# NVIDIA/makani

Hardware: AMD Instinct MI355X
Metric: SFNO train samples/sec at 721x1440x73ch (higher is better)
Workload: dtype bf16; 1 GPU; sfno_sc3_layers8_edim384; grid=721x1440, channels=73, global_batch=1, parallelism=dp1, spectral_arithmetic=x3, multistep_count=1, multistep_checkpoint=False, launch=hipGraph replay of the captured step, channel_gemm=hip (csrc/conv1x1.hip)

## Files before the change

### include/makani_amd.h

```cpp
#ifndef MAKANI_AMD_H
#define MAKANI_AMD_H

#ifdef __cplusplus
extern "C" {
#endif

#define MK_F32 0
#define MK_BF16 1

#define MK_EINVAL -1
#define MK_EUNSUP -2

#define MK_TRI_NONE 0
#define MK_TRI_ROW_GE 1
#define MK_TRI_K_GE 2
#define MK_TRI_ROW_LE 3
#define MK_TRI_K_LE 4

typedef struct MkGemm {
    const float* A;
    const float* B;
    float* C;
    long long a_batch, a_row, a_k;
    long long b_batch, b_col, b_k;
// ... 92 lines not shown

long long mk_spec_lp_blocks(int L, int M);
int mk_spec_lp_fwd(const float* S, const float* wgt, float* partial, int L, int M, long long R, int tri_off, int m_off,
                   float p, float w0, float w1, void* stream);
int mk_spec_lp_bwd(const float* S, const float* wgt, const float* g, float* dS, int L, int M, long long R, int tri_off,
                   int m_off, float p, float w0, float w1, void* stream);

int mk_spec_sep_mul(const float* x, const float* w, float* y, int L, int M, int Mw, int B, int Cp, int tri_off, int conj_w,
                    void* stream);
int mk_spec_sep_wgrad(const float* x, const float* gy, float* gw, int L, int M, int Mw, int B, int Cp, int tri_off, void* stream);
int mk_spec_diag_apply(const float* x, const float* w_c64, float* y, int L, int M, int B, int Cin, int Cout, int x_ld, int y_ld,
                       int y_pad, int tri_off, int dgrad, void* stream);
int mk_spec_diag_wgrad(const float* x, const float* gy, float* gw_c64, int L, int M, int B, int Cin, int Cout, int x_ld, int y_ld,
                       int tri_off, void* stream);

int mk_conv1x1_nn(const void* A, const void* X, void* Y, void* Ypre, const float* bias, const void* R, const void* G,
                  int M, int K, int lda, int B, long long N, int act, void* stream);
long long mk_conv1x1_wgrad_workspace(int M, int K, int B, long long N);
int mk_conv1x1_wgrad(const void* G, const void* X, float* dW, float* part, int M, int K, int B, long long N,
                     int accumulate, void* stream);
int mk_conv1x1_wgrad_fuses_bias(int M, int K, int B, long long N);
int mk_conv1x1_wgrad_bias(const void* G, const void* X, float* dW, float* dbias, float* part, int M, int K, int B, long long N,
                          int accumulate, void* stream);

int mk_adamw_step(float* p, const float* g, float* m, float* v, long long n, const float* grad_scale, float lr,
                  float beta1, float beta2, float eps, float weight_decay, int step, const float* step_state, void* stream);
int mk_adamw_advance(float* state, float beta1, float beta2, void* stream);
typedef struct MkAdamTensor {
    float* p;
    const float* g;
    float* m;
    float* v;
    long long n;
    void* p_bf16;
    void* p_bf16_t;
    int cols;
    int ld, ld_t;
} MkAdamTensor;
int mk_adamw_multi(const MkAdamTensor* tensors, int count, const float* grad_scale, float lr, float beta1, float beta2,
                   float eps, float weight_decay, int step, const float* step_state, void* stream);
long long mk_grad_norm_workspace(const MkAdamTensor* tensors, int count);
int mk_grad_clip_coef(const MkAdamTensor* tensors, int count, float max_norm, float* partial, float* out, void* stream);
long long mk_grad_norm_workspace_pre(const MkAdamTensor* tensors, int count, const MkAdamTensor* pre, int npre);
int mk_grad_clip_coef_pre(const MkAdamTensor* tensors, int count, const MkAdamTensor* pre, int npre, float max_norm, float* partial,
                          float* out, void* stream);

// ... 111 lines not shown
```

### makani_amd/_lib.py

```python
import ctypes as C
import os

import torch

_HERE = os.path.dirname(os.path.abspath(__file__))
LIB_PATH = os.environ.get("MAKANI_AMD_LIB") or os.path.join(_HERE, "libmakani_amd.so")

MK_F32, MK_BF16 = 0, 1
TRI_NONE, TRI_ROW_GE, TRI_K_GE, TRI_ROW_LE, TRI_K_LE = 0, 1, 2, 3, 4

c_ll, c_int, c_f, c_vp = C.c_longlong, C.c_int, C.c_float, C.c_void_p


class MkAdamTensor(C.Structure):
    _fields_ = [("p", C.c_void_p), ("g", C.c_void_p), ("m", C.c_void_p), ("v", C.c_void_p), ("n", C.c_longlong),
                ("p_bf16", C.c_void_p), ("p_bf16_t", C.c_void_p), ("cols", C.c_int), ("ld", C.c_int), ("ld_t", C.c_int)]


class MkGemm(C.Structure):
    _fields_ = [
        ("A", c_vp), ("B", c_vp), ("C", c_vp),
        ("a_batch", c_ll), ("a_row", c_ll), ("a_k", c_ll),
        ("b_batch", c_ll), ("b_col", c_ll), ("b_k", c_ll),
        ("c_batch", c_ll), ("c_row", c_ll), ("c_col", c_ll),
        ("a_inner", c_ll), ("b_inner", c_ll), ("c_inner", c_ll),
        ("a_im", c_ll), ("b_im", c_ll), ("c_im", c_ll),
        ("M", c_int), ("N", c_int), ("K", c_int), ("batch", c_int),
        ("inner", c_int), ("tri_mode", c_int), ("tri_off", c_int),
        ("conj_a", c_int), ("conj_b", c_int), ("beta", c_int),
    ]


MK_FFT_SEG_MAX = 8


class MkFftSeg(C.Structure):
    _fields_ = [("nw", c_int), ("nh", c_int), ("m_off", c_int * (MK_FFT_SEG_MAX + 1)), ("r_off", c_int * (MK_FFT_SEG_MAX + 1)),
                ("base", (c_ll * MK_FFT_SEG_MAX) * MK_FFT_SEG_MAX), ("xseg", c_int), ("x_stride", c_ll), ("x_nlat", c_int)]

# ... 24 lines not shown
    "mk_spec_sep_mul": ([c_vp, c_vp, c_vp, c_int, c_int, c_int, c_int, c_int, c_int, c_int, c_vp], c_int),
    "mk_spec_sep_wgrad": ([c_vp, c_vp, c_vp, c_int, c_int, c_int, c_int, c_int, c_int, c_vp], c_int),
    "mk_spec_diag_apply": ([c_vp, c_vp, c_vp, c_int, c_int, c_int, c_int, c_int, c_int, c_int, c_int, c_int, c_int, c_vp], c_int),
    "mk_spec_diag_wgrad": ([c_vp, c_vp, c_vp, c_int, c_int, c_int, c_int, c_int, c_int, c_int, c_int, c_vp], c_int),
    "mk_pointwise_chunks": ([c_ll, c_int, c_ll], c_int),
    "mk_plane_sums": ([c_vp, c_int, c_vp, c_vp, c_ll, c_ll, c_vp], c_int),
    "mk_instnorm_stats": ([c_vp, c_int, c_vp, c_vp, c_ll, c_ll, c_f, c_vp, c_f, c_vp], c_int),
    "mk_instnorm_merge": ([c_vp, c_vp, c_vp, c_ll, c_int, c_f, c_vp], c_int),
    "mk_instnorm_apply": ([c_vp, c_vp, c_int, c_vp, c_vp, c_vp, c_ll, c_int, c_ll, c_int, c_vp], c_int),
    "mk_instnorm_fused_chunks": ([c_ll, c_int, c_ll, c_int], c_int),
    "mk_instnorm_fwd_fused": ([c_vp, c_vp, c_int, c_vp, c_vp, c_vp, c_vp, c_vp, c_vp, c_ll, c_int, c_ll, c_f, c_int, c_vp], c_int),
    "mk_instnorm_bwd_fused": ([c_vp, c_vp, c_vp, c_int, c_vp, c_vp, c_vp, c_vp, c_vp, c_vp, c_vp, c_ll, c_int, c_ll, c_int, c_vp], c_int),
    "mk_instnorm_bwd": ([c_vp, c_vp, c_vp, c_int, c_vp, c_vp, c_vp, c_vp, c_vp, c_f, c_vp, c_vp, c_ll, c_int, c_ll, c_ll, c_int, c_int, c_vp], c_int),
    "mk_chan_layernorm_chunks": ([c_int, c_ll], c_int),
    "mk_chan_layernorm_fwd": ([c_vp, c_int, c_vp, c_int, c_vp, c_vp, c_vp, c_int, c_int, c_ll, c_f, c_vp], c_int),
    "mk_chan_layernorm_bwd": ([c_vp, c_int, c_vp, c_int, c_vp, c_vp, c_vp, c_int, c_int, c_ll, c_vp], c_int),
    "mk_chan_layernorm_wgrad": ([c_vp, c_int, c_vp, c_int, c_vp, c_vp, c_int, c_int, c_ll, c_vp], c_int),
    "mk_bias_gelu_fwd": ([c_vp, c_vp, c_vp, c_int, c_ll, c_int, c_ll, c_vp], c_int),
    "mk_conv1x1_nn": ([c_vp, c_vp, c_vp, c_vp, c_vp, c_vp, c_vp, c_int, c_int, c_int, c_int, c_ll, c_int, c_vp], c_int),
    "mk_conv1x1_wgrad_workspace": ([c_int, c_int, c_int, c_ll], c_ll),
    "mk_conv1x1_wgrad": ([c_vp, c_vp, c_vp, c_vp, c_int, c_int, c_int, c_ll, c_int, c_vp], c_int),
    "mk_conv1x1_wgrad_fuses_bias": ([c_int, c_int, c_int, c_ll], c_int),
    "mk_conv1x1_wgrad_bias": ([c_vp, c_vp, c_vp, c_vp, c_vp, c_int, c_int, c_int, c_ll, c_int, c_vp], c_int),
    "mk_adamw_step": ([c_vp, c_vp, c_vp, c_vp, c_ll, c_vp, c_f, c_f, c_f, c_f, c_f, c_int, c_vp, c_vp], c_int),
    "mk_adamw_advance": ([c_vp, c_f, c_f, c_vp], c_int),
    "mk_bias_gelu_bwd": ([c_vp, c_vp, c_vp, c_vp, c_vp, c_vp, c_int, c_ll, c_int, c_ll, c_vp], c_int),
    "mk_adamw_multi": ([c_vp, c_int, c_vp, c_f, c_f, c_f, c_f, c_f, c_int, c_vp, c_vp], c_int),
    "mk_instnorm_fwd": ([c_vp, c_vp, c_int, c_vp, c_vp, c_vp, c_vp, c_vp, c_vp, c_f, c_ll, c_int, c_ll, c_f, c_int, c_vp], c_int),
    "mk_grad_norm_workspace": ([c_vp, c_int], c_ll),
    "mk_grad_clip_coef": ([c_vp, c_int, c_f, c_vp, c_vp, c_vp], c_int),
    "mk_grad_norm_workspace_pre": ([c_vp, c_int, c_vp, c_int], c_ll),
    "mk_grad_clip_coef_pre": ([c_vp, c_int, c_vp, c_int, c_f, c_vp, c_vp, c_vp], c_int),
    "mk_spec_lp_blocks": ([c_int, c_int], c_ll),
    "mk_spec_lp_fwd": ([c_vp, c_vp, c_vp, c_int, c_int, c_ll, c_int, c_int, c_f, c_f, c_f, c_vp], c_int),
    "mk_spec_lp_bwd": ([c_vp, c_vp, c_vp, c_vp, c_int, c_int, c_ll, c_int, c_int, c_f, c_f, c_f, c_vp], c_int),
    "mk_crps_chunks": ([c_ll], c_int),
    "mk_crps": ([c_vp, c_int, c_vp, c_int, c_vp, c_vp, c_vp, c_vp, c_vp, c_int, c_int, c_int, c_ll, c_int, c_f, c_f, c_int, c_vp, c_vp], c_int),
    "mk_crps_complex": ([c_vp, c_vp, c_vp, c_vp, c_vp, c_vp, c_vp, c_int, c_int, c_int, c_ll, c_f, c_int, c_vp], c_int),
    "mk_escore_sums_workspace": ([c_int, c_int, c_int, c_ll, c_int, c_int], c_ll),
    "mk_escore_sums": ([c_vp, c_int, c_vp, c_vp, c_vp, c_vp, c_vp, c_int, c_int, c_int, c_ll, c_int, c_int, c_f, c_vp], c_int),
    "mk_escore_finish": ([c_vp, c_vp, c_int, c_vp, c_vp, c_int, c_int, c_int, c_int, c_int, c_f, c_f, c_f, c_f, c_vp], c_int),
    "mk_escore_grad": ([c_vp, c_int, c_vp, c_vp, c_vp, c_vp, c_vp, c_vp, c_int, c_int, c_int, c_int, c_ll, c_int, c_int, c_f, c_vp], c_int),
    "mk_mmd_finish": ([c_vp, c_vp, c_vp, c_int, c_int, c_int, c_int, c_f, c_f, c_vp], c_int),
    "mk_amse_sums": ([c_vp, c_vp, c_vp, c_vp, c_ll, c_int, c_int, c_int, c_int, c_vp], c_int),
    "mk_amse_grad": ([c_vp, c_vp, c_vp, c_vp, c_vp, c_vp, c_ll, c_int, c_int, c_int, c_int, c_vp], c_int),
    "mk_ens_nll_chunks": ([c_ll], c_int),
# ... 124 lines not shown
```

### makani_amd/csrc/conv1x1.hip

```cpp
#include <stdlib.h>
#include <type_traits>

#include "common.h"
#include "conv1x1_plan.h"

#ifndef MK_ASTAT_DIAG
#define MK_ASTAT_DIAG 0
#endif
#if MK_ASTAT_DIAG
__device__ unsigned long long g_astat_diag[16];
#define MK_AS_STAMP(k)                                              \
    do {                                                            \
        const unsigned long long t_ = __builtin_readcyclecounter(); \
        dg[k] += t_ - tprev;                                        \
        tprev = t_;                                                 \
    } while (0)
#else
#define MK_AS_STAMP(k)
#endif

namespace {

typedef __bf16 bf16x8 __attribute__((ext_vector_type(8)));
typedef __attribute__((address_space(3))) s16x4 lds_s16x4;
// ... 1364 lines not shown
    for (int i = 0; i < 2; ++i)
#pragma unroll
        for (int j = 0; j < 2; ++j) {
            const int c = c0 + wn * 64 + j * 32 + l31;
#pragma unroll
            for (int r = 0; r < 16; ++r) {
                const int m = m0 + wm * 64 + i * 32 + (r & 3) + 8 * (r >> 2) + 4 * lh;
                if (m < p.M && c < p.K) out[(long long)m * p.K + c] = acc[i][j][r];
            }
        }
}

struct ConvWgR {
    const u16* P;
    const u16* Q;
    float* part;
    int RP, RQ, B, S, slabs, qslabs;
    int ldo;
    long long N;
    long long chunk;
    float* bias_part;
};


template <int WP, int WQ, int WTP, int WTQ, bool SWAP>
__global__ __launch_bounds__(512, 2) void conv_wgrad_ring_kernel(const ConvWgR p) {
#if defined(__HIP_DEVICE_COMPILE__)
    static_assert(WP * WQ == 8, "8 waves");
    constexpr int TP = WP * WTP * 32, TQ = WQ * WTQ * 32;
    constexpr int BK = 64;
    constexpr int STAGE = (TP + TQ) * 128;
    constexpr int NI = (TP + TQ) / 64;
    constexpr int NIP = TP / 64;
    static_assert(TP % 64 == 0 && TQ == 384, "row groups; Q is fetched by 2 x 3 DMA pieces per wave");
    __shared__ __attribute__((aligned(1024))) unsigned char smem[2 * STAGE];

    const int bid = xcd_remap(blockIdx.x, gridDim.x);
    const int slab = bid % p.slabs;
    const int qs = (bid / p.slabs) % p.qslabs;
    const int q0 = qs * TQ;
    const int sp = bid / (p.slabs * p.qslabs);
    const int splits_per_b = p.S / p.B;
    const int b = sp / splits_per_b;
    const long long nbeg = (long long)(sp % splits_per_b) * p.chunk;
    const long long nend = min(p.N, nbeg + p.chunk);
    const int nk = nbeg < nend ? (int)((nend - nbeg + BK - 1) / BK) : 0;

    const int tid = threadIdx.x, lane = tid & 63, wave = tid >> 6;
    const int wp = wave / WQ, wq = wave % WQ;
    const int l31 = lane & 31, lh = lane >> 5;

    const int c_log = (lane & 7) ^ ((((wave & 1) << 2) + (lane >> 4)) & 7);
    const unsigned rowbytes = (unsigned)(p.N * 2);
    unsigned voff[NI];
#pragma unroll
    for (int i = 0; i < NI; ++i) {
        const int rg = wave + 8 * i;
        int row;
        if (i < NIP) row = min(rg * 8 + (lane >> 3), p.RP - 1 - slab * TP);
        else row = min((rg - TP / 8) * 8 + (lane >> 3), p.RQ - 1 - q0);
        voff[i] = (unsigned)row * rowbytes + (unsigned)c_log * 16u;
    }
    const v4i_t rsP = make_rsrc(p.P + ((long long)b * p.RP + slab * TP) * p.N);
    const v4i_t rsQ = make_rsrc(p.Q + ((long long)b * p.RQ + q0) * p.N);
// ... 87 lines not shown
            const int m = SWAP ? q0 + (wq * WTQ + i) * 32 + l31 : slab * TP + (wp * WTP + i) * 32 + l31;
            if (lh == 0 && m < RG) p.bias_part[((long long)sp * NSH + bshare) * RG + m] = tot;
        }
    }

    float* out = p.part + (long long)sp * ((long long)(SWAP ? p.RQ : p.RP) * p.ldo);
#pragma unroll
    for (int i = 0; i < WTP; ++i)
#pragma unroll
        for (int j = 0; j < WTQ; ++j) {
            const int prow0 = slab * TP + (wp * WTP + i) * 32, qrow0 = q0 + (wq * WTQ + j) * 32;
#pragma unroll
            for (int r = 0; r < 16; ++r) {
                const int rr = (r & 3) + 8 * (r >> 2) + 4 * lh;
                const int m = SWAP ? qrow0 + rr : prow0 + rr;
                const int k = SWAP ? prow0 + l31 : qrow0 + l31;
                const bool ok = SWAP ? (m < p.RQ && k < p.RP) : (m < p.RP && k < p.RQ);
                if (ok) out[(long long)m * p.ldo + k] = acc[i][j][r];
            }
        }
#endif
}

__global__ void reduce_splits(const float* __restrict__ part, float* __restrict__ out, long long n, int S, int accumulate) {
    const long long i = (long long)blockIdx.x * blockDim.x + threadIdx.x;
    if (i >= n) return;
    float s = accumulate ? out[i] : 0.f;
    int k = 0;
    for (; k + 8 <= S; k += 8) {
        float v[8];
#pragma unroll
        for (int u = 0; u < 8; ++u) v[u] = part[(long long)(k + u) * n + i];
#pragma unroll
        for (int u = 0; u < 8; ++u) s += v[u];
    }
    for (; k < S; ++k) s += part[(long long)k * n + i];
    out[i] = s;
}

__global__ void reduce_splits4(const float4* __restrict__ part, float4* __restrict__ out, long long n4, int S, int accumulate) {
    const long long i = (long long)blockIdx.x * blockDim.x + threadIdx.x;
    if (i >= n4) return;
    float4 s = accumulate ? out[i] : make_float4(0.f, 0.f, 0.f, 0.f);
    int k = 0;
    for (; k + 8 <= S; k += 8) {
        float4 v[8];
#pragma unroll
        for (int u = 0; u < 8; ++u) v[u] = part[(long long)(k + u) * n4 + i];
#pragma unroll
        for (int u = 0; u < 8; ++u) s.x += v[u].x, s.y += v[u].y, s.z += v[u].z, s.w += v[u].w;
    }
    for (; k < S; ++k) {
        const float4 v = part[(long long)k * n4 + i];
        s.x += v.x, s.y += v.y, s.z += v.z, s.w += v.w;
    }
    out[i] = s;
}

}

#if MK_ASTAT_DIAG
extern "C" int mk_astat_diag_read(unsigned long long* out, int reset) {
    if (hipMemcpyFromSymbol(out, HIP_SYMBOL(g_astat_diag), sizeof(unsigned long long) * 16) != hipSuccess) return 1;
    if (reset) {
        unsigned long long z[16] = {};
        if (hipMemcpyToSymbol(HIP_SYMBOL(g_astat_diag), z, sizeof(z)) != hipSuccess) return 1;
    }
    return 0;
}
#endif

static int env_int(const char* name) {
    const char* e = getenv(name);
    return e ? atoi(e) : -1;
}

extern "C" int mk_conv1x1_nn(const void* A, const void* X, void* Y, void* Ypre, const float* bias, const void* R,
                             const void* G, int M, int K, int lda, int B, long long N, int act, void* stream) {
    MK_REQUIRE(A && X && Y, "conv1x1_nn: null pointer");
// ... 50 lines not shown
        const long long tn = (N + 255) / 256;
        const long long nt = (long long)tm * tn * B;
        const unsigned grid = (unsigned)(nt < 256 ? nt : 256);
        if (bm == 384) hipLaunchKernelGGL((conv_nn_ring_kernel<6>), dim3(grid), dim3(512), 0, s, p, tm, tn, nt);
        else if (bm == 256) hipLaunchKernelGGL((conv_nn_ring_kernel<4>), dim3(grid), dim3(512), 0, s, p, tm, tn, nt);
        else hipLaunchKernelGGL((conv_nn_ring_kernel<3>), dim3(grid), dim3(512), 0, s, p, tm, tn, nt);
        break;
    }
    case ConvNnKernel::tile: {
        constexpr int BM = 128;
        const int tm = (M + BM - 1) / BM;
        const int BN = N >= (1ll << 19) ? 256 : 128;
        const long long tn = (N + BN - 1) / BN;
        const long long nb = (long long)tm * tn * B;
        MK_REQUIRE(nb < (1ll << 31), "conv1x1_nn: grid too large");
        if (BN == 256) hipLaunchKernelGGL((conv_nn_kernel<BM, 256, 1, 64, 2>), dim3((unsigned)nb), dim3(NT), 0, s, p, tm, tn);
        else hipLaunchKernelGGL((conv_nn_kernel<BM, 128, 1, 64, 3>), dim3((unsigned)nb), dim3(NT), 0, s, p, tm, tn);
        break;
    }
    }
    return mk_check_launch("mk_conv1x1_nn");
}

namespace {
struct WgPlan {
    bool ring;
    bool swap;
    int tp;
    int slabs;
    int qslabs;
    long long S;
    long long chunk;
};

WgPlan wgrad_plan(int M, int K, int B, long long N) {
    WgPlan pl{};
    const int big = M > K ? M : K, small = M > K ? K : M;
    if (big >= 96 && N * 2 * 384 < (1ll << 31) && N >= 2048) {
        pl.ring = true;
        int q, pr;
        if (big <= 384) { q = big; pr = small; }
        else if (small <= 384) { q = small; pr = big; }
        else { q = big; pr = small; }
        const bool q_is_x = (K == q) && !(M == q && M > K);
        pl.swap = !q_is_x;
        pl.tp = (pr > 192 && pr % 256 != 192 && (pr % 192 != 0 || pr % 256 == 0)) ? 256 : 192;
        if (pr <= 192) pl.tp = 192;
        pl.slabs = (pr + pl.tp - 1) / pl.tp;
        pl.qslabs = (q + 383) / 384;
        long long per_b = 256 / ((long long)pl.slabs * pl.qslabs * B);
        if (per_b < 1) per_b = 1;
        const long long maxs = (N + 511) / 512;
        if (per_b > maxs) per_b = maxs;
        long long chunk = ((N + per_b - 1) / per_b + 63) / 64 * 64;
        per_b = (N + chunk - 1) / chunk;
        pl.chunk = chunk;
        pl.S = per_b * B;
        return pl;
    }
    const int tiles = ((M + 127) / 128) * ((K + 127) / 128);
    long long per_b = 1024 / ((long long)tiles * B);
    if (per_b < 1) per_b = 1;
    const long long maxs = (N + 2047) / 2048;
    if (per_b > maxs) per_b = maxs;
    long long chunk = (N + per_b - 1) / per_b;
    chunk = (chunk + 127) / 128 * 128;
    pl.chunk = chunk;
    pl.S = per_b * B;
    return pl;
}
}

extern "C" long long mk_conv1x1_wgrad_workspace(int M, int K, int B, long long N) {
    const WgPlan pl = wgrad_plan(M, K, B, N);
    return pl.S * (long long)M * K + pl.S * (long long)M;
}

extern "C" int mk_conv1x1_wgrad_fuses_bias(int M, int K, int B, long long N) {
    return wgrad_plan(M, K, B, N).ring ? 1 : 0;
}

static int conv1x1_wgrad_impl(const void* G, const void* X, float* dW, float* dbias, float* part, int M, int K, int B, long long N,
                              int accumulate, void* stream);

extern "C" int mk_conv1x1_wgrad(const void* G, const void* X, float* dW, float* part, int M, int K, int B, long long N,
                                int accumulate, void* stream) {
    return conv1x1_wgrad_impl(G, X, dW, nullptr, part, M, K, B, N, accumulate, stream);
}

extern "C" int mk_conv1x1_wgrad_bias(const void* G, const void* X, float* dW, float* dbias, float* part, int M, int K, int B,
                                     long long N, int accumulate, void* stream) {
    MK_REQUIRE(dbias, "conv1x1_wgrad_bias: null pointer");
    MK_REQUIRE(wgrad_plan(M, K, B, N).ring, "conv1x1_wgrad_bias: this shape runs the tile kernel, which does not form the bias gradient");
    return conv1x1_wgrad_impl(G, X, dW, dbias, part, M, K, B, N, accumulate, stream);
}

static int conv1x1_wgrad_impl(const void* G, const void* X, float* dW, float* dbias, float* part, int M, int K, int B, long long N,
                              int accumulate, void* stream) {
    MK_REQUIRE(G && X && dW && part, "conv1x1_wgrad: null pointer");
    MK_REQUIRE(M > 0 && K > 0 && B > 0 && N > 0 && (N % 8) == 0, "conv1x1_wgrad: bad shape");
    const WgPlan pl = wgrad_plan(M, K, B, N);
    hipStream_t s = (hipStream_t)stream;
    if (pl.ring) {
        ConvWgR p{};
        p.P = (const u16*)(pl.swap ? X : G);
        p.Q = (const u16*)(pl.swap ? G : X);
        p.RP = pl.swap ? K : M;
        p.RQ = pl.swap ? M : K;
        p.part = part, p.B = B, p.S = (int)pl.S, p.slabs = pl.slabs, p.qslabs = pl.qslabs, p.ldo = K, p.N = N, p.chunk = pl.chunk;
        p.bias_part = dbias ? part + pl.S * (long long)M * K : nullptr;
        const dim3 grid((unsigned)(pl.slabs * pl.qslabs * pl.S)), blk(512);
        if (pl.tp == 256) {
            if (pl.swap) hipLaunchKernelGGL((conv_wgrad_ring_kernel<2, 4, 4, 3, true>), grid, blk, 0, s, p);
            else hipLaunchKernelGGL((conv_wgrad_ring_kernel<2, 4, 4, 3, false>), grid, blk, 0, s, p);
        } else {
            if (pl.swap) hipLaunchKernelGGL((conv_wgrad_ring_kernel<2, 4, 3, 3, true>), grid, blk, 0, s, p);
            else hipLaunchKernelGGL((conv_wgrad_ring_kernel<2, 4, 3, 3, false>), grid, blk, 0, s, p);
        }
    } else {
        const int tm = (M + 127) / 128, tk = (K + 127) / 128;
        ConvWg p{(const u16*)G, (const u16*)X, part, M, K, B, (int)pl.S, N, pl.chunk};
        hipLaunchKernelGGL(conv_wgrad_kernel<128>, dim3((unsigned)(tm * tk * pl.S)), dim3(NT), 0, s, p, tm, tk);
    }
    const long long n = (long long)M * K;
    if (n % 4 == 0 && (((uintptr_t)part | (uintptr_t)dW) & 15) == 0)
        hipLaunchKernelGGL(reduce_splits4, dim3((unsigned)((n / 4 + 255) / 256)), dim3(256), 0, s, (const float4*)part, (float4*)dW,
                           n / 4, (int)pl.S, accumulate);
    else
        hipLaunchKernelGGL(reduce_splits, dim3((unsigned)((n + 255) / 256)), dim3(256), 0, s, part, dW, n, (int)pl.S, accumulate);
    if (dbias)
        hipLaunchKernelGGL(reduce_splits, dim3((unsigned)((M + 255) / 256)), dim3(256), 0, s, part + pl.S * n, dbias, (long long)M,
                           (int)pl.S, 0);
    return mk_check_launch("mk_conv1x1_wgrad");
}
```

### makani_amd/csrc/conv1x1_plan.h

```cpp
#pragma once

enum class ConvNnKernel {
    astat73,
    astat2,
    astat1,
    ring,
    tile
};

inline ConvNnKernel conv_nn_plan(int M, int K, int lda, int B, long long N, bool pre, bool has_r, bool has_g, int astat2_env) {
    const bool stationary = M >= 256 && (long long)M * N * 2 < (1ll << 31) && N >= 64 && !(has_r && has_g);
    if (stationary && lda == 80 && K > 64 && K <= 80 && (long long)K * N * 2 < (1ll << 32) && !((has_r || has_g) && pre))
        return ConvNnKernel::astat73;
    const bool small_ring = M == 384 && (long long)B * N <= 32768 && !pre && astat2_env != 1;
    if (stationary && K == 384 && !small_ring) return astat2_env == 0 ? ConvNnKernel::astat1 : ConvNnKernel::astat2;
    if (K >= 64 && M >= 192 && N * 2 * 64 < (1ll << 31) && (long long)M * lda * 2 < (1ll << 31) && N >= 256) return ConvNnKernel::ring;
    return ConvNnKernel::tile;
}

inline int conv_nn_ring_rows(int M, int K, int B, long long N, bool has_epilogue, int ring384_env) {
    const int rows = ((M % 256 == 0) || M > 576) ? 256 : 192;
    const long long tiles384 = ((N + 255) / 256) * B;
    if (rows == 192 && M > 192 && M <= 384 && K >= 512 && !has_epilogue && tiles384 >= 256 && ring384_env != 0) return 384;
    return rows;
}
```

### makani_amd/ops.py

```python
import ctypes as C
import os
import weakref
from dataclasses import dataclass

import numpy as np
import torch

from . import _lib
from ._lib import MkGemm, check, dtype_code, lib, ptr, stream
from . import legendre as _leg


def round4(n: int) -> int:
    return (n + 3) // 4 * 4


GEMM_MODE = os.environ.get("MAKANI_AMD_GEMM", "auto")
if GEMM_MODE not in ("auto", "x6", "x3", "fp32"):
    raise ValueError(f"MAKANI_AMD_GEMM={GEMM_MODE!r}: expected auto, x6, x3 or fp32")


def gemm_mode() -> str:
    if GEMM_MODE != "auto":
        return GEMM_MODE
# ... 985 lines not shown
    return y, ypre


def conv1x1_wgrad(g: torch.Tensor, x: torch.Tensor, want_bias: bool = False):
    B, M, H, W = g.shape
    K = x.shape[1]
    N = H * W
    g, x = g.contiguous(), x.contiguous()
    nws = lib().mk_conv1x1_wgrad_workspace(M, K, B, N)
    part = torch.empty((nws,), dtype=torch.float32, device=g.device)
    dW = torch.empty((M, K), dtype=torch.float32, device=g.device)
    fused = want_bias and bool(lib().mk_conv1x1_wgrad_fuses_bias(M, K, B, N))
    with _timed(f"conv1x1_wgrad_m{M}_k{K}_n{N}", flops=2.0 * B * M * K * N, nbytes=2.0 * B * N * (M + K)):
        if fused:
            db = torch.empty((M,), dtype=torch.float32, device=g.device)
            check(lib().mk_conv1x1_wgrad_bias(ptr(g), ptr(x), ptr(dW), ptr(db), ptr(part), M, K, B, N, 0, stream()), "mk_conv1x1_wgrad_bias")
        else:
            check(lib().mk_conv1x1_wgrad(ptr(g), ptr(x), ptr(dW), ptr(part), M, K, B, N, 0, stream()), "mk_conv1x1_wgrad")
    if not want_bias:
        return dW
    return dW, (db if fused else _sum_planes(g))


def _sum_planes(t: torch.Tensor) -> torch.Tensor:
    if not (t.is_cuda and t.dim() == 4 and t.dtype in (torch.bfloat16, torch.float32)):
        raise RuntimeError("makani_amd ops need 4-d bf16 / fp32 GPU tensors (the HIP path has no CPU fallback)")
    t = t.contiguous()
    B, Cc, H, W = t.shape
    sums = torch.empty((2, B * Cc), dtype=torch.float32, device=t.device)
    check(lib().mk_plane_sums(ptr(t), dtype_code(t), ptr(sums), ptr(_ws(B * Cc, H * W, t.dtype, t.device)), B * Cc, H * W,
                              stream()), "mk_plane_sums")
    return _batch_sum(sums, B, Cc)[0]


class Conv1x1Fn(torch.autograd.Function):

    @staticmethod
    def forward(ctx, x, weight, bias, residual):
        M, K = weight.shape[0], weight.shape[1]
        A, At = weight_operands(weight, need_t=ctx.needs_input_grad[0])
        y, _ = conv1x1_nn(A, K, x, bias=bias, residual=residual)
        ctx.save_for_backward(x, weight, At)
        ctx.has_bias = bias is not None
        ctx.has_res = residual is not None
        return y

# ... 22 lines not shown
class ConvGeluConvFn(torch.autograd.Function):

    @staticmethod
    def forward(ctx, x, w1, b1, w2, b2):
        H1, K = w1.shape[0], w1.shape[1]
        M = w2.shape[0]
        A1, A1t = weight_operands(w1, need_t=ctx.needs_input_grad[0])
        A2, A2t = weight_operands(w2, need_t=True)
        h, a1 = conv1x1_nn(A1, K, x, bias=b1, act=True, want_pre=True)
        y, _ = conv1x1_nn(A2, H1, h, bias=b2)
        ctx.save_for_backward(x, w1, w2, a1, h, A1t, A2t)
        ctx.has_b = (b1 is not None, b2 is not None)
        return y

    @staticmethod
    def backward(ctx, gy):
        x, w1, w2, a1, h, A1t, A2t = ctx.saved_tensors
        H1, K = w1.shape[0], w1.shape[1]
        M = w2.shape[0]
        gy = gy.contiguous()
        ga1, _ = conv1x1_nn(A2t, M, gy, gelu_grad_of=a1)
        gw2 = gb2 = gw1 = gb1 = None
        want_b2, want_b1 = ctx.has_b[1] and ctx.needs_input_grad[4], ctx.has_b[0] and ctx.needs_input_grad[2]
        if ctx.needs_input_grad[3] and want_b2:
            gw2, gb2 = conv1x1_wgrad(gy, h, want_bias=True)
            gw2 = gw2.view_as(w2)
        else:
            gw2 = conv1x1_wgrad(gy, h).view_as(w2) if ctx.needs_input_grad[3] else None
            gb2 = _sum_planes(gy) if want_b2 else None
        if ctx.needs_input_grad[1] and want_b1:
            gw1, gb1 = conv1x1_wgrad(ga1, x, want_bias=True)
            gw1 = gw1.view_as(w1)
        else:
            gw1 = conv1x1_wgrad(ga1, x).view_as(w1) if ctx.needs_input_grad[1] else None
            gb1 = _sum_planes(ga1) if want_b1 else None
        gx = None
        if ctx.needs_input_grad[0]:
            gx, _ = conv1x1_nn(A1t, H1, ga1)
        return gx, gw1, gb1, gw2, gb2


def want_bf16_shadow(param):
    param._mk_want_bf16 = True


def _shadow_valid(weight):
    return (getattr(weight, "_mk_shadow", None) is not None and getattr(weight, "_mk_shadow_version", -1) == weight._version
            and getattr(weight, "_mk_shadow_ptr", 0) == weight.data_ptr() and weight._mk_shadow.device == weight.device)


def cast_weight(weight, dtype):
    if dtype == weight.dtype:
        return weight
    if dtype == torch.bfloat16 and _shadow_valid(weight):
        K = weight.numel() // weight.shape[0]
        sh = weight._mk_shadow
        return sh.view(weight.shape) if sh.shape[1] == K else sh[:, :K]
    return weight.to(dtype)
# ... 245 lines not shown
```

Before: 27.68 samples/s.

## Batch both MLP weight-gradient GEMMs into one grouped ring kernel launch

Adds a grouped weight-gradient entry point that puts the two conv1x1 wgrad problems of the MLP backward into a single ring-kernel grid. Each block finds its problem and tile from a flattened tile index, and the split count is planned over the combined tile total. The split reductions for weights and biases are merged into one multi-segment reduce kernel. The aim is fewer launches and better occupancy for small per-problem grids, at the cost of a shared split plan and a larger workspace.

```diff
diff --git a/include/makani_amd.h b/include/makani_amd.h
--- a/include/makani_amd.h
+++ b/include/makani_amd.h
@@ -138,6 +138,16 @@
 int mk_conv1x1_wgrad_fuses_bias(int M, int K, int B, long long N);
 int mk_conv1x1_wgrad_bias(const void* G, const void* X, float* dW, float* dbias, float* part, int M, int K, int B, long long N,
                           int accumulate, void* stream);
+typedef struct MkWgradProblem {
+    const void* G;
+    const void* X;
+    float* dW;
+    float* dbias;
+    int M, K;
+    int accumulate;
+} MkWgradProblem;
+long long mk_conv1x1_wgrad_multi_workspace(const MkWgradProblem* probs, int n, int B, long long N);
+int mk_conv1x1_wgrad_multi(const MkWgradProblem* probs, int n, float* part, int B, long long N, void* stream);
 
 int mk_adamw_step(float* p, const float* g, float* m, float* v, long long n, const float* grad_scale, float lr,
                   float beta1, float beta2, float eps, float weight_decay, int step, const float* step_state, void* stream);
diff --git a/makani_amd/_lib.py b/makani_amd/_lib.py
--- a/makani_amd/_lib.py
+++ b/makani_amd/_lib.py
@@ -15,6 +15,11 @@
 class MkAdamTensor(C.Structure):
     _fields_ = [("p", C.c_void_p), ("g", C.c_void_p), ("m", C.c_void_p), ("v", C.c_void_p), ("n", C.c_longlong),
                 ("p_bf16", C.c_void_p), ("p_bf16_t", C.c_void_p), ("cols", C.c_int), ("ld", C.c_int), ("ld_t", C.c_int)]
+
+
+class MkWgradProblem(C.Structure):
+    _fields_ = [("G", C.c_void_p), ("X", C.c_void_p), ("dW", C.c_void_p), ("dbias", C.c_void_p), ("M", C.c_int), ("K", C.c_int),
+                ("accumulate", C.c_int)]
 
 
 class MkGemm(C.Structure):
@@ -85,6 +90,8 @@
     "mk_conv1x1_wgrad": ([c_vp, c_vp, c_vp, c_vp, c_int, c_int, c_int, c_ll, c_int, c_vp], c_int),
     "mk_conv1x1_wgrad_fuses_bias": ([c_int, c_int, c_int, c_ll], c_int),
     "mk_conv1x1_wgrad_bias": ([c_vp, c_vp, c_vp, c_vp, c_vp, c_int, c_int, c_int, c_ll, c_int, c_vp], c_int),
+    "mk_conv1x1_wgrad_multi_workspace": ([C.POINTER(MkWgradProblem), c_int, c_int, c_ll], c_ll),
+    "mk_conv1x1_wgrad_multi": ([C.POINTER(MkWgradProblem), c_int, c_vp, c_int, c_ll, c_vp], c_int),
     "mk_adamw_step": ([c_vp, c_vp, c_vp, c_vp, c_ll, c_vp, c_f, c_f, c_f, c_f, c_f, c_int, c_vp, c_vp], c_int),
     "mk_adamw_advance": ([c_vp, c_f, c_f, c_vp], c_int),
     "mk_bias_gelu_bwd": ([c_vp, c_vp, c_vp, c_vp, c_vp, c_vp, c_int, c_ll, c_int, c_ll, c_vp], c_int),
diff --git a/makani_amd/csrc/conv1x1.hip b/makani_amd/csrc/conv1x1.hip
--- a/makani_amd/csrc/conv1x1.hip
+++ b/makani_amd/csrc/conv1x1.hip
@@ -1410,9 +1410,23 @@
     float* bias_part;
 };
 
+struct ConvWgProb {
+    const u16* P;
+    const u16* Q;
+    float* part;
+    float* bias_part;
+    int RP, RQ, slabs, qslabs, ldo, swap;
+};
+struct ConvWgM {
+    ConvWgProb pr[WG_MULTI_MAX];
+    int n, T, B, S;
+    long long N;
+    long long chunk;
+};
+
 
 template <int WP, int WQ, int WTP, int WTQ, bool SWAP>
-__global__ __launch_bounds__(512, 2) void conv_wgrad_ring_kernel(const ConvWgR p) {
+__device__ __forceinline__ void conv_wgrad_ring_tile(const ConvWgR& p, unsigned char* smem, const int slab, const int qs, const int sp) {
 #if defined(__HIP_DEVICE_COMPILE__)
     static_assert(WP * WQ == 8, "8 waves");
     constexpr int TP = WP * WTP * 32, TQ = WQ * WTQ * 32;
@@ -1421,13 +1435,8 @@
     constexpr int NI = (TP + TQ) / 64;
     constexpr int NIP = TP / 64;
     static_assert(TP % 64 == 0 && TQ == 384, "row groups; Q is fetched by 2 x 3 DMA pieces per wave");
-    __shared__ __attribute__((aligned(1024))) unsigned char smem[2 * STAGE];
-
-    const int bid = xcd_remap(blockIdx.x, gridDim.x);
-    const int slab = bid % p.slabs;
-    const int qs = (bid / p.slabs) % p.qslabs;
+
     const int q0 = qs * TQ;
-    const int sp = bid / (p.slabs * p.qslabs);
     const int splits_per_b = p.S / p.B;
     const int b = sp / splits_per_b;
     const long long nbeg = (long long)(sp % splits_per_b) * p.chunk;
@@ -1561,39 +1570,90 @@
 #endif
 }
 
-__global__ void reduce_splits(const float* __restrict__ part, float* __restrict__ out, long long n, int S, int accumulate) {
-    const long long i = (long long)blockIdx.x * blockDim.x + threadIdx.x;
-    if (i >= n) return;
-    float s = accumulate ? out[i] : 0.f;
-    int k = 0;
-    for (; k + 8 <= S; k += 8) {
-        float v[8];
-#pragma unroll
-        for (int u = 0; u < 8; ++u) v[u] = part[(long long)(k + u) * n + i];
-#pragma unroll
-        for (int u = 0; u < 8; ++u) s += v[u];
-    }
-    for (; k < S; ++k) s += part[(long long)k * n + i];
-    out[i] = s;
-}
-
-__global__ void reduce_splits4(const float4* __restrict__ part, float4* __restrict__ out, long long n4, int S, int accumulate) {
-    const long long i = (long long)blockIdx.x * blockDim.x + threadIdx.x;
-    if (i >= n4) return;
-    float4 s = accumulate ? out[i] : make_float4(0.f, 0.f, 0.f, 0.f);
-    int k = 0;
-    for (; k + 8 <= S; k += 8) {
-        float4 v[8];
-#pragma unroll
-        for (int u = 0; u < 8; ++u) v[u] = part[(long long)(k + u) * n4 + i];
-#pragma unroll
-        for (int u = 0; u < 8; ++u) s.x += v[u].x, s.y += v[u].y, s.z += v[u].z, s.w += v[u].w;
-    }
-    for (; k < S; ++k) {
-        const float4 v = part[(long long)k * n4 + i];
-        s.x += v.x, s.y += v.y, s.z += v.z, s.w += v.w;
-    }
-    out[i] = s;
+template <int WTP>
+__global__ __launch_bounds__(512, 2) void conv_wgrad_ring_kernel(const ConvWgM a) {
+#if defined(__HIP_DEVICE_COMPILE__)
+    constexpr int STAGE = (2 * WTP * 32 + 384) * 128;
+    __shared__ __attribute__((aligned(1024))) unsigned char smem[2 * STAGE];
+    const int bid = xcd_remap(blockIdx.x, gridDim.x);
+    int t = bid % a.T;
+    const int sp = bid / a.T;
+    int i = 0;
+    for (; i + 1 < a.n; ++i) {
+        const int nt = a.pr[i].slabs * a.pr[i].qslabs;
+        if (t < nt) break;
+        t -= nt;
+    }
+    const ConvWgProb& q = a.pr[i];
+    ConvWgR p;
+    p.P = q.P, p.Q = q.Q, p.part = q.part, p.bias_part = q.bias_part;
+    p.RP = q.RP, p.RQ = q.RQ, p.slabs = q.slabs, p.qslabs = q.qslabs, p.ldo = q.ldo;
+    p.B = a.B, p.S = a.S, p.N = a.N, p.chunk = a.chunk;
+    const int slab = __builtin_amdgcn_readfirstlane(t % q.slabs), qs = __builtin_amdgcn_readfirstlane(t / q.slabs);
+    if (q.swap) conv_wgrad_ring_tile<2, 4, WTP, 3, true>(p, smem, slab, qs, sp);
+    else conv_wgrad_ring_tile<2, 4, WTP, 3, false>(p, smem, slab, qs, sp);
+#endif
+}
+
+struct RedSeg {
+    const float* part;
+    float* out;
+    long long n;
+    int vec, accumulate;
+    unsigned blk0;
+};
+struct RedArgs {
+    RedSeg seg[2 * WG_MULTI_MAX];
+    int nseg, S;
+};
+
+__global__ __launch_bounds__(256) void reduce_splits_multi(const RedArgs a) {
+    int g = 0;
+    while (g + 1 < a.nseg && blockIdx.x >= a.seg[g + 1].blk0) ++g;
+    const RedSeg& sg = a.seg[g];
+    const long long i = (long long)(blockIdx.x - sg.blk0) * 256 + threadIdx.x;
+    if (i >= sg.n) return;
+    const int S = a.S;
+    if (sg.vec) {
+        const float4* part = (const float4*)sg.part;
+        float4* out = (float4*)sg.out;
+        const long long n4 = sg.n;
+        float4 s = sg.accumulate ? out[i] : make_float4(0.f, 0.f, 0.f, 0.f);
+        int k = 0;
+        for (; k + 8 <= S; k += 8) {
+            float4 v[8];
+#pragma unroll
+            for (int u = 0; u < 8; ++u) v[u] = part[(long long)(k + u) * n4 + i];
+#pragma unroll
+            for (int u = 0; u < 8; ++u) s.x += v[u].x, s.y += v[u].y, s.z += v[u].z, s.w += v[u].w;
+        }
+        for (; k < S; ++k) {
+            const float4 v = part[(long long)k * n4 + i];
+            s.x += v.x, s.y += v.y, s.z += v.z, s.w += v.w;
+        }
+        out[i] = s;
+    } else {
+        const float* part = sg.part;
+        const long long n = sg.n;
+        float s = sg.accumulate ? sg.out[i] : 0.f;
+        int k = 0;
+        for (; k + 8 <= S; k += 8) {
+            float v[8];
+#pragma unroll
+            for (int u = 0; u < 8; ++u) v[u] = part[(long long)(k + u) * n + i];
+#pragma unroll
+            for (int u = 0; u < 8; ++u) s += v[u];
+        }
+        for (; k < S; ++k) s += part[(long long)k * n + i];
+        sg.out[i] = s;
+    }
+}
+
+inline void red_add(RedArgs& a, unsigned& blocks, const float* part, float* out, long long n, int accumulate) {
+    RedSeg& sg = a.seg[a.nseg++];
+    const bool vec = n % 4 == 0 && (((uintptr_t)part | (uintptr_t)out) & 15) == 0;
+    sg.part = part, sg.out = out, sg.n = vec ? n / 4 : n, sg.vec = vec, sg.accumulate = accumulate, sg.blk0 = blocks;
+    blocks += (unsigned)((sg.n + 255) / 256);
 }
 
 }
@@ -1690,55 +1750,6 @@
     return mk_check_launch("mk_conv1x1_nn");
 }
 
-namespace {
-struct WgPlan {
-    bool ring;
-    bool swap;
-    int tp;
-    int slabs;
-    int qslabs;
-    long long S;
-    long long chunk;
-};
-
-WgPlan wgrad_plan(int M, int K, int B, long long N) {
-    WgPlan pl{};
-    const int big = M > K ? M : K, small = M > K ? K : M;
-    if (big >= 96 && N * 2 * 384 < (1ll << 31) && N >= 2048) {
-        pl.ring = true;
-        int q, pr;
-        if (big <= 384) { q = big; pr = small; }
-        else if (small <= 384) { q = small; pr = big; }
-        else { q = big; pr = small; }
-        const bool q_is_x = (K == q) && !(M == q && M > K);
-        pl.swap = !q_is_x;
-        pl.tp = (pr > 192 && pr % 256 != 192 && (pr % 192 != 0 || pr % 256 == 0)) ? 256 : 192;
-        if (pr <= 192) pl.tp = 192;
-        pl.slabs = (pr + pl.tp - 1) / pl.tp;
-        pl.qslabs = (q + 383) / 384;
-        long long per_b = 256 / ((long long)pl.slabs * pl.qslabs * B);
-        if (per_b < 1) per_b = 1;
-        const long long maxs = (N + 511) / 512;
-        if (per_b > maxs) per_b = maxs;
-        long long chunk = ((N + per_b - 1) / per_b + 63) / 64 * 64;
-        per_b = (N + chunk - 1) / chunk;
-        pl.chunk = chunk;
-        pl.S = per_b * B;
-        return pl;
-    }
-    const int tiles = ((M + 127) / 128) * ((K + 127) / 128);
-    long long per_b = 1024 / ((long long)tiles * B);
-    if (per_b < 1) per_b = 1;
-    const long long maxs = (N + 2047) / 2048;
-    if (per_b > maxs) per_b = maxs;
-    long long chunk = (N + per_b - 1) / per_b;
-    chunk = (chunk + 127) / 128 * 128;
-    pl.chunk = chunk;
-    pl.S = per_b * B;
-    return pl;
-}
-}
-
 extern "C" long long mk_conv1x1_wgrad_workspace(int M, int K, int B, long long N) {
     const WgPlan pl = wgrad_plan(M, K, B, N);
     return pl.S * (long long)M * K + pl.S * (long long)M;
@@ -1761,6 +1772,38 @@
     MK_REQUIRE(dbias, "conv1x1_wgrad_bias: null pointer");
     MK_REQUIRE(wgrad_plan(M, K, B, N).ring, "conv1x1_wgrad_bias: this shape runs the tile kernel, which does not form the bias gradient");
     return conv1x1_wgrad_impl(G, X, dW, dbias, part, M, K, B, N, accumulate, stream);
+}
+
+static void wgrad_ring_launch(const MkWgradProblem* probs, const WgPlan* pl, int n, int tp, long long S, long long chunk, float* part,
+                              int B, long long N, hipStream_t s) {
+    ConvWgM a{};
+    RedArgs r{};
+    unsigned rblocks = 0;
+    a.n = n, a.B = B, a.S = (int)S, a.N = N, a.chunk = chunk;
+    float* w = part;
+    for (int i = 0; i < n; ++i) {
+        const MkWgradProblem& q = probs[i];
+        ConvWgProb& d = a.pr[i];
+        d.P = (const u16*)(pl[i].swap ? q.X : q.G);
+        d.Q = (const u16*)(pl[i].swap ? q.G : q.X);
+        d.RP = pl[i].swap ? q.K : q.M;
+        d.RQ = pl[i].swap ? q.M : q.K;
+        d.slabs = pl[i].slabs, d.qslabs = pl[i].qslabs, d.ldo = q.K, d.swap = pl[i].swap;
+        d.part = w;
+        a.T += d.slabs * d.qslabs;
+        red_add(r, rblocks, w, q.dW, (long long)q.M * q.K, q.accumulate);
+        w += S * (long long)q.M * q.K;
+    }
+    for (int i = 0; i < n; ++i) {
+        a.pr[i].bias_part = probs[i].dbias ? w : nullptr;
+        if (probs[i].dbias) red_add(r, rblocks, w, probs[i].dbias, (long long)probs[i].M, 0);
+        w += S * (long long)probs[i].M;
+    }
+    r.S = (int)S;
+    const dim3 grid((unsigned)(a.T * S)), blk(512);
+    if (tp == 256) hipLaunchKernelGGL((conv_wgrad_ring_kernel<4>), grid, blk, 0, s, a);
+    else hipLaunchKernelGGL((conv_wgrad_ring_kernel<3>), grid, blk, 0, s, a);
+    hipLaunchKernelGGL(reduce_splits_multi, dim3(rblocks), dim3(256), 0, s, r);
 }
 
 static int conv1x1_wgrad_impl(const void* G, const void* X, float* dW, float* dbias, float* part, int M, int K, int B, long long N,
@@ -1770,34 +1813,55 @@
     const WgPlan pl = wgrad_plan(M, K, B, N);
     hipStream_t s = (hipStream_t)stream;
     if (pl.ring) {
-        ConvWgR p{};
-        p.P = (const u16*)(pl.swap ? X : G);
-        p.Q = (const u16*)(pl.swap ? G : X);
-        p.RP = pl.swap ? K : M;
-        p.RQ = pl.swap ? M : K;
-        p.part = part, p.B = B, p.S = (int)pl.S, p.slabs = pl.slabs, p.qslabs = pl.qslabs, p.ldo = K, p.N = N, p.chunk = pl.chunk;
-        p.bias_part = dbias ? part + pl.S * (long long)M * K : nullptr;
-        const dim3 grid((unsigned)(pl.slabs * pl.qslabs * pl.S)), blk(512);
-        if (pl.tp == 256) {
-            if (pl.swap) hipLaunchKernelGGL((conv_wgrad_ring_kernel<2, 4, 4, 3, true>), grid, blk, 0, s, p);
-            else hipLaunchKernelGGL((conv_wgrad_ring_kernel<2, 4, 4, 3, false>), grid, blk, 0, s, p);
-        } else {
-            if (pl.swap) hipLaunchKernelGGL((conv_wgrad_ring_kernel<2, 4, 3, 3, true>), grid, blk, 0, s, p);
-            else hipLaunchKernelGGL((conv_wgrad_ring_kernel<2, 4, 3, 3, false>), grid, blk, 0, s, p);
-        }
+        const MkWgradProblem q{G, X, dW, dbias, M, K, accumulate};
+        wgrad_ring_launch(&q, &pl, 1, pl.tp, pl.S, pl.chunk, part, B, N, s);
     } else {
         const int tm = (M + 127) / 128, tk = (K + 127) / 128;
         ConvWg p{(const u16*)G, (const u16*)X, part, M, K, B, (int)pl.S, N, pl.chunk};
         hipLaunchKernelGGL(conv_wgrad_kernel<128>, dim3((unsigned)(tm * tk * pl.S)), dim3(NT), 0, s, p, tm, tk);
-    }
-    const long long n = (long long)M * K;
-    if (n % 4 == 0 && (((uintptr_t)part | (uintptr_t)dW) & 15) == 0)
-        hipLaunchKernelGGL(reduce_splits4, dim3((unsigned)((n / 4 + 255) / 256)), dim3(256), 0, s, (const float4*)part, (float4*)dW,
-                           n / 4, (int)pl.S, accumulate);
-    else
-        hipLaunchKernelGGL(reduce_splits, dim3((unsigned)((n + 255) / 256)), dim3(256), 0, s, part, dW, n, (int)pl.S, accumulate);
-    if (dbias)
-        hipLaunchKernelGGL(reduce_splits, dim3((unsigned)((M + 255) / 256)), dim3(256), 0, s, part + pl.S * n, dbias, (long long)M,
-                           (int)pl.S, 0);
+        RedArgs r{};
+        unsigned rblocks = 0;
+        red_add(r, rblocks, part, dW, (long long)M * K, accumulate);
+        r.S = (int)pl.S;
+        hipLaunchKernelGGL(reduce_splits_multi, dim3(rblocks), dim3(256), 0, s, r);
+    }
     return mk_check_launch("mk_conv1x1_wgrad");
 }
+
+static bool wgrad_multi_shapes(const MkWgradProblem* probs, int n, int* M, int* K) {
+    if (!probs || n < 1 || n > WG_MULTI_MAX) return false;
+    for (int i = 0; i < n; ++i) {
+        M[i] = probs[i].M, K[i] = probs[i].K;
+        if (M[i] <= 0 || K[i] <= 0) return false;
+    }
+    return true;
+}
+
+extern "C" long long mk_conv1x1_wgrad_multi_workspace(const MkWgradProblem* probs, int n, int B, long long N) {
+    int M[WG_MULTI_MAX], K[WG_MULTI_MAX];
+    MK_REQUIRE(wgrad_multi_shapes(probs, n, M, K) && B > 0 && N > 0, "conv1x1_wgrad_multi_workspace: 1 to %d problems of positive shape", WG_MULTI_MAX);
+    return wgrad_multi_workspace(M, K, n, B, N);
+}
+
+extern "C" int mk_conv1x1_wgrad_multi(const MkWgradProblem* probs, int n, float* part, int B, long long N, void* stream) {
+    int M[WG_MULTI_MAX], K[WG_MULTI_MAX];
+    MK_REQUIRE(wgrad_multi_shapes(probs, n, M, K), "conv1x1_wgrad_multi: 1 to %d problems of positive shape", WG_MULTI_MAX);
+    MK_REQUIRE(part && B > 0 && N > 0 && (N % 8) == 0, "conv1x1_wgrad_multi: bad shape");
+    const WgMultiPlan mp = wgrad_multi_plan(M, K, n, B, N);
+    for (int i = 0; i < n; ++i) {
+        MK_REQUIRE(probs[i].G && probs[i].X && probs[i].dW, "conv1x1_wgrad_multi: null pointer");
+        MK_REQUIRE(!probs[i].dbias || mp.p[i].ring,
+                   "conv1x1_wgrad_multi: problem %d runs the tile kernel, which does not form the bias gradient", i);
+    }
+    if (mp.paired) {
+        wgrad_ring_launch(probs, mp.p, n, mp.tp, mp.S, mp.chunk, part, B, N, (hipStream_t)stream);
+        return mk_check_launch("mk_conv1x1_wgrad_multi");
+    }
+    for (int i = 0; i < n; ++i) {
+        const MkWgradProblem& q = probs[i];
+        const int rc = conv1x1_wgrad_impl(q.G, q.X, q.dW, q.dbias, part, q.M, q.K, B, N, q.accumulate, stream);
+        if (rc) return rc;
+        part += mp.p[i].S * (long long)q.M * q.K + mp.p[i].S * (long long)q.M;
+    }
+    return 0;
+}
diff --git a/makani_amd/csrc/conv1x1_plan.h b/makani_amd/csrc/conv1x1_plan.h
--- a/makani_amd/csrc/conv1x1_plan.h
+++ b/makani_amd/csrc/conv1x1_plan.h
@@ -24,3 +24,87 @@
     if (rows == 192 && M > 192 && M <= 384 && K >= 512 && !has_epilogue && tiles384 >= 256 && ring384_env != 0) return 384;
     return rows;
 }
+
+struct WgPlan {
+    bool ring;
+    bool swap;
+    int tp;
+    int slabs;
+    int qslabs;
+    long long S;
+    long long chunk;
+};
+
+inline void wgrad_ring_splits(long long tiles, int B, long long N, long long* S, long long* chunk_out) {
+    long long per_b = 256 / (tiles * B);
+    if (per_b < 1) per_b = 1;
+    const long long maxs = (N + 511) / 512;
+    if (per_b > maxs) per_b = maxs;
+    const long long chunk = ((N + per_b - 1) / per_b + 63) / 64 * 64;
+    per_b = (N + chunk - 1) / chunk;
+    *chunk_out = chunk;
+    *S = per_b * B;
+}
+
+inline WgPlan wgrad_plan(int M, int K, int B, long long N) {
+    WgPlan pl{};
+    const int big = M > K ? M : K, small = M > K ? K : M;
+    if (big >= 96 && N * 2 * 384 < (1ll << 31) && N >= 2048) {
+        pl.ring = true;
+        int q, pr;
+        if (big <= 384) { q = big; pr = small; }
+        else if (small <= 384) { q = small; pr = big; }
+        else { q = big; pr = small; }
+        const bool q_is_x = (K == q) && !(M == q && M > K);
+        pl.swap = !q_is_x;
+        pl.tp = (pr > 192 && pr % 256 != 192 && (pr % 192 != 0 || pr % 256 == 0)) ? 256 : 192;
+        if (pr <= 192) pl.tp = 192;
+        pl.slabs = (pr + pl.tp - 1) / pl.tp;
+        pl.qslabs = (q + 383) / 384;
+        wgrad_ring_splits((long long)pl.slabs * pl.qslabs, B, N, &pl.S, &pl.chunk);
+        return pl;
+    }
+    const int tiles = ((M + 127) / 128) * ((K + 127) / 128);
+    long long per_b = 1024 / ((long long)tiles * B);
+    if (per_b < 1) per_b = 1;
+    const long long maxs = (N + 2047) / 2048;
+    if (per_b > maxs) per_b = maxs;
+    long long chunk = (N + per_b - 1) / per_b;
+    chunk = (chunk + 127) / 128 * 128;
+    pl.chunk = chunk;
+    pl.S = per_b * B;
+    return pl;
+}
+
+constexpr int WG_MULTI_MAX = 3;
+struct WgMultiPlan {
+    bool paired;
+    int tp;
+    int T;
+    long long S;
+    long long chunk;
+    WgPlan p[WG_MULTI_MAX];
+};
+
+inline WgMultiPlan wgrad_multi_plan(const int* M, const int* K, int n, int B, long long N) {
+    WgMultiPlan mp{};
+    for (int i = 0; i < n && i < WG_MULTI_MAX; ++i) mp.p[i] = wgrad_plan(M[i], K[i], B, N);
+    if (n < 2 || n > WG_MULTI_MAX) return mp;
+    for (int i = 0; i < n; ++i)
+        if (!mp.p[i].ring || mp.p[i].tp != mp.p[0].tp) return mp;
+    mp.paired = true;
+    mp.tp = mp.p[0].tp;
+    for (int i = 0; i < n; ++i) mp.T += mp.p[i].slabs * mp.p[i].qslabs;
+    wgrad_ring_splits(mp.T, B, N, &mp.S, &mp.chunk);
+    return mp;
+}
+
+inline long long wgrad_multi_workspace(const int* M, const int* K, int n, int B, long long N) {
+    const WgMultiPlan mp = wgrad_multi_plan(M, K, n, B, N);
+    long long w = 0;
+    for (int i = 0; i < n && i < WG_MULTI_MAX; ++i) {
+        const long long S = mp.paired ? mp.S : mp.p[i].S;
+        w += S * (long long)M[i] * K[i] + S * (long long)M[i];
+    }
+    return w;
+}
diff --git a/makani_amd/ops.py b/makani_amd/ops.py
--- a/makani_amd/ops.py
+++ b/makani_amd/ops.py
@@ -1031,6 +1031,35 @@
     return dW, (db if fused else _sum_planes(g))
 
 
+WGRAD_PAIR = os.environ.get("MAKANI_AMD_WGRAD_PAIR", "1") != "0"
+
+
+def conv1x1_wgrad_multi(problems):
+    B, _, H, W = problems[0][0].shape
+    N = H * W
+    dev = problems[0][0].device
+    keep, out = [], []
+    arr = (_lib.MkWgradProblem * len(problems))()
+    for i, (g, x, want_bias) in enumerate(problems):
+        M, K = g.shape[1], x.shape[1]
+        assert g.shape[0] == B == x.shape[0] and g.shape[2:] == (H, W) == x.shape[2:]
+        g, x = g.contiguous(), x.contiguous()
+        fused = want_bias and bool(lib().mk_conv1x1_wgrad_fuses_bias(M, K, B, N))
+        dW = torch.empty((M, K), dtype=torch.float32, device=dev)
+        db = torch.empty((M,), dtype=torch.float32, device=dev) if fused else None
+        arr[i] = _lib.MkWgradProblem(ptr(g), ptr(x), ptr(dW), ptr(db), M, K, 0)
+        keep.append((g, x))
+        out.append((dW, db, want_bias and not fused))
+    nws = lib().mk_conv1x1_wgrad_multi_workspace(arr, len(problems), B, N)
+    if nws < 0:
+        check(int(nws), "mk_conv1x1_wgrad_multi_workspace")
+    part = torch.empty((nws,), dtype=torch.float32, device=dev)
+    Ms, Ks = sum(p.M for p in arr), sum(p.K for p in arr)
+    with _timed(f"conv1x1_wgrad_m{Ms}_k{Ks}_n{N}", flops=2.0 * B * N * sum(p.M * p.K for p in arr), nbytes=2.0 * B * N * (Ms + Ks)):
+        check(lib().mk_conv1x1_wgrad_multi(arr, len(problems), ptr(part), B, N, stream()), "mk_conv1x1_wgrad_multi")
+    return [(dW, _sum_planes(g) if plane else db) for (dW, db, plane), (g, _) in zip(out, keep)]
+
+
 def _sum_planes(t: torch.Tensor) -> torch.Tensor:
     if not (t.is_cuda and t.dim() == 4 and t.dtype in (torch.bfloat16, torch.float32)):
         raise RuntimeError("makani_amd ops need 4-d bf16 / fp32 GPU tensors (the HIP path has no CPU fallback)")
@@ -1099,18 +1128,22 @@
         ga1, _ = conv1x1_nn(A2t, M, gy, gelu_grad_of=a1)
         gw2 = gb2 = gw1 = gb1 = None
         want_b2, want_b1 = ctx.has_b[1] and ctx.needs_input_grad[4], ctx.has_b[0] and ctx.needs_input_grad[2]
-        if ctx.needs_input_grad[3] and want_b2:
-            gw2, gb2 = conv1x1_wgrad(gy, h, want_bias=True)
-            gw2 = gw2.view_as(w2)
+        if WGRAD_PAIR and ctx.needs_input_grad[3] and ctx.needs_input_grad[1]:
+            (gw2, gb2), (gw1, gb1) = conv1x1_wgrad_multi([(gy, h, want_b2), (ga1, x, want_b1)])
+            gw2, gw1 = gw2.view_as(w2), gw1.view_as(w1)
         else:
-            gw2 = conv1x1_wgrad(gy, h).view_as(w2) if ctx.needs_input_grad[3] else None
-            gb2 = _sum_planes(gy) if want_b2 else None
-        if ctx.needs_input_grad[1] and want_b1:
-            gw1, gb1 = conv1x1_wgrad(ga1, x, want_bias=True)
-            gw1 = gw1.view_as(w1)
-        else:
-            gw1 = conv1x1_wgrad(ga1, x).view_as(w1) if ctx.needs_input_grad[1] else None
-            gb1 = _sum_planes(ga1) if want_b1 else None
+            if ctx.needs_input_grad[3] and want_b2:
+                gw2, gb2 = conv1x1_wgrad(gy, h, want_bias=True)
+                gw2 = gw2.view_as(w2)
+            else:
+                gw2 = conv1x1_wgrad(gy, h).view_as(w2) if ctx.needs_input_grad[3] else None
+                gb2 = _sum_planes(gy) if want_b2 else None
+            if ctx.needs_input_grad[1] and want_b1:
+                gw1, gb1 = conv1x1_wgrad(ga1, x, want_bias=True)
+                gw1 = gw1.view_as(w1)
+            else:
+                gw1 = conv1x1_wgrad(ga1, x).view_as(w1) if ctx.needs_input_grad[1] else None
+                gb1 = _sum_planes(ga1) if want_b1 else None
         gx = None
         if ctx.needs_input_grad[0]:
             gx, _ = conv1x1_nn(A1t, H1, ga1)
```

Result: no change. 27.93 samples/s (median of 6 runs) (+0.9%).
